# chengzhag/PanFusion

Measured on NVIDIA H100. Metric: denoise-steps/sec (512x1024 pano + 8x512^2 views, 50-step DDIM), higher is better.
Workload: dtype bf16

## Files before the change

### panfusion_b200/csrc/gemm_common.cuh

```cuda
#pragma once
#include "pf_common.cuh"

namespace pf {

constexpr int GEMM_BLOCK_M = 128;
constexpr int GEMM_BLOCK_K = 64;
constexpr int GEMM_WIN_SPAN = 8;
constexpr int GEMM_WIN_BYTES = (GEMM_BLOCK_M + GEMM_WIN_SPAN) * GEMM_BLOCK_K * 2;

struct GemmKernelParams {
  int M, N, kb_per_tap;
  int num_groups, num_units;
  int grp_first[PF_MAX_TAPS + 1];
  int grp_off[PF_MAX_TAPS];
  int tap_src[PF_MAX_TAPS];
  int a_rows, a_slots, slab_ring;
  unsigned long long grp_shifts[PF_MAX_TAPS];
  void* out;
  int out_ld;
  int out_f32;
  const float* bias;
  const float* rowbias;
  int rowbias_ld;
  int rows_per_group;
  const void* residual;
  int res_ld;
  int res_f32;
  int act;
  int map_mode, Hm, Wm, i0, j0, Hout, Wout;
  int osy, osx, oa, ob;
  int k_splits;
  float* ws;
  float* row_stats;
  int stat_slots;
  const float* ln_stats;
  int ln_slots;
  const float* ln_colsum;
  float ln_inv_k, ln_eps;
};

__device__ __forceinline__ void ln_row_coeffs(const GemmKernelParams& p, long long m, float& a, float& b) {
  const float4* st = reinterpret_cast<const float4*>(p.ln_stats) + m * (p.ln_slots >> 1);
  const int pairs = p.ln_slots >> 1;
  float s = 0.f, q = 0.f;
  for (int i0 = 0; i0 < pairs; i0 += 4) {
    float4 v[4];
#pragma unroll
    for (int u = 0; u < 4; ++u) v[u] = i0 + u < pairs ? __ldg(st + i0 + u) : make_float4(0.f, 0.f, 0.f, 0.f);
#pragma unroll
    for (int u = 0; u < 4; ++u) {
      s += v[u].x;
      q += v[u].y;
      s += v[u].z;
      q += v[u].w;
    }
  }
  const float mean = s * p.ln_inv_k;
  const float var = fmaxf(q * p.ln_inv_k - mean * mean, 0.f);
  a = rsqrtf(var + p.ln_eps);
  b = -mean * a;
}

__host__ __device__ constexpr int gemm_stage_bytes(int block_n) {
  return GEMM_BLOCK_M * GEMM_BLOCK_K * 2 + block_n * GEMM_BLOCK_K * 2;
}

}
```

### panfusion_b200/csrc/gemm_wgmma.cu

```cuda
#include <stdlib.h>

#include "gemm_common.cuh"
#include "wgmma.cuh"

namespace pf {

constexpr int GEMM_THREADS = 256;

constexpr int GEMM_SUB_BYTES = GEMM_BLOCK_M * 64;
constexpr int GEMM_SMEM_CORESIDENT = 228 * 1024 / 2 - 1024;

__host__ __device__ constexpr int gemm_acc_ld(int block_n) { return block_n + 4; }
__host__ __device__ constexpr int gemm_acc_bytes(int block_n) {
  return (GEMM_BLOCK_M * gemm_acc_ld(block_n) * 4 + 1023) / 1024 * 1024;
}
__host__ __device__ constexpr int gemm_ring_bytes(int block_n, int stages, bool epi_tma) {
  const int ring = stages * gemm_stage_bytes(block_n);
  const int epi = gemm_acc_bytes(block_n) + (epi_tma ? 2 * GEMM_SUB_BYTES : 0);
  return ((ring > epi ? ring : epi) + 1023) / 1024 * 1024;
}
__host__ __device__ constexpr int gemm_bar_bytes(int stages) { return (2 * stages * 12 + 15) / 16 * 16; }
__host__ __device__ constexpr int gemm_smem_bytes(int block_n, int stages, bool epi_tma) {
  return gemm_ring_bytes(block_n, stages, epi_tma) + gemm_bar_bytes(stages) +
         2 * block_n * 4 ;
}

template <int BLOCK_N, int STAGES, int CTAS, bool BF16, bool EPI_TMA>
__global__ void __launch_bounds__(GEMM_THREADS, CTAS)
gemm_taps_kernel(const __grid_constant__ CUtensorMap tmA, const __grid_constant__ CUtensorMap tmB,
                 const __grid_constant__ CUtensorMap tmC, const GemmKernelParams p) {
  constexpr int B_BYTES = BLOCK_N * GEMM_BLOCK_K * 2;
  constexpr int RING_BYTES = gemm_ring_bytes(BLOCK_N, STAGES, EPI_TMA);
  constexpr int ACC_LD = gemm_acc_ld(BLOCK_N);
  constexpr int NCH = BLOCK_N / 16;
  constexpr int NACC = BLOCK_N / 2;
  static_assert(BLOCK_N % 32 == 0 && BLOCK_N <= 256, "tile width");

  extern __shared__ __align__(1024) uint8_t smem[];
  if ((smem_u32(smem) & 1023u) != 0) __trap();
  float* sacc = reinterpret_cast<float*>(smem);
  uint8_t* staging = smem + gemm_acc_bytes(BLOCK_N);
  const int a_bytes = p.a_rows * (GEMM_BLOCK_K * 2);
  uint8_t* const b_ring = smem + p.a_slots * a_bytes;
  uint64_t* a_full = reinterpret_cast<uint64_t*>(smem + RING_BYTES);
  uint64_t* b_full = a_full + STAGES;
  uint32_t* a_rel = reinterpret_cast<uint32_t*>(b_full + STAGES);
  uint32_t* b_rel = a_rel + STAGES;
  float* s_bias = reinterpret_cast<float*>(smem + RING_BYTES + gemm_bar_bytes(STAGES));
  float* s_cs = s_bias + BLOCK_N;

  const int et = threadIdx.x;
  const int lane = et & 31;
  const int wg = et >> 7;
  const int n_tiles = p.N / BLOCK_N;
  const int n_tile = int(blockIdx.x) % n_tiles;
  const int m0 = (int(blockIdx.x) / n_tiles) * GEMM_BLOCK_M;
  const int n0 = n_tile * BLOCK_N;
  const int kpt = p.kb_per_tap;
  const int split = p.k_splits > 1 ? int(blockIdx.y) : 0;
  const int u_begin = (p.k_splits > 1) ? (int)((long long)split * p.num_units / p.k_splits) : 0;
  const int u_end = (p.k_splits > 1) ? (int)((long long)(split + 1) * p.num_units / p.k_splits) : p.num_units;
  auto first_slab = [&](int u) {
    const int gu = u / kpt, ku = u - gu * kpt;
    return p.grp_first[gu] * kpt + (ku ? ku * (p.grp_first[gu + 1] - p.grp_first[gu]) : 0);
  };
  const int s_begin = first_slab(u_begin), s_end = first_slab(u_end);

  if (et == 0) {
    tma_prefetch_desc(&tmA);
    tma_prefetch_desc(&tmB);
    for (int s = 0; s < STAGES; ++s) {
      mbar_init(&a_full[s], 1);
      mbar_init(&b_full[s], 1);
      a_rel[s] = b_rel[s] = 0u;
    }
    if constexpr (EPI_TMA) tma_prefetch_desc(&tmC);
    fence_barrier_init();
  }
  __syncthreads();

  auto locate = [&](int s, int& gs, int& ks, int& is) {
    gs = 0;
    while (s >= p.grp_first[gs + 1] * kpt) ++gs;
    const int taps = p.grp_first[gs + 1] - p.grp_first[gs];
    const int r = s - p.grp_first[gs] * kpt;
    ks = r / taps;
    is = p.grp_first[gs] + r - ks * taps;
  };
  auto load_a = [&](int slot, int ga, int ka, uint64_t* bar) {
    tma_load_2d(smem + slot * a_bytes, &tmA, bar, ka * GEMM_BLOCK_K, m0 + p.grp_off[ga]);
  };
  auto fill_a = [&](int slot, int ga, int ka) {
    mbar_expect_tx(&a_full[slot], a_bytes);
    load_a(slot, ga, ka, &a_full[slot]);
  };
  auto fill_b = [&](int slot, int gb, int kb, int ib) {
    mbar_expect_tx(&b_full[slot], B_BYTES + (p.slab_ring ? a_bytes : 0));
    if (p.slab_ring) load_a(slot, gb, kb, &b_full[slot]);
    tma_load_2d(b_ring + slot * B_BYTES, &tmB, &b_full[slot], (p.tap_src[ib] * kpt + kb) * GEMM_BLOCK_K, n0);
  };
  if (et == 0) {
    if (!p.slab_ring)
      for (int k = 0; k < p.a_slots && u_begin + k < u_end; ++k) {
        const int gu = (u_begin + k) / kpt;
        fill_a(k, gu, u_begin + k - gu * kpt);
      }
    for (int k = 0; k < STAGES && s_begin + k < s_end; ++k) {
      int gs, ks, is;
      locate(s_begin + k, gs, ks, is);
      fill_b(k, gs, ks, is);
    }
  }
  auto released_last = [](uint32_t* counter) {
    __threadfence_block();
    const uint32_t before = atomicAdd(counter, 1u);
    __threadfence_block();
    return (before & 1u) != 0u;
  };

  if (p.bias && et < BLOCK_N) s_bias[et] = __ldg(p.bias + n0 + et);
  if (p.ln_stats && et < BLOCK_N) s_cs[et] = __ldg(p.ln_colsum + n0 + et);
  {
    float acc[NACC];
#pragma unroll
    for (int i = 0; i < NACC; ++i) acc[i] = 0.f;
    int g = u_begin / kpt, kk = u_begin - g * kpt, t = 0;
    int gsize = p.grp_first[g + 1] - p.grp_first[g];
    uint64_t gshift = p.grp_shifts[g];
    int a_slot = 0, a_par = 0, b_slot = 0, b_par = 0;
    int gb = 0, kb = 0, ib = 0;
    if (s_begin + STAGES < s_end) locate(s_begin + STAGES, gb, kb, ib);
    int ib0 = p.grp_first[gb], ib_end = p.grp_first[gb + 1];
    int ua = u_begin + p.a_slots, ga = ua / kpt, ka = ua - ga * kpt;
    auto issue_slab = [&]() {
      if (!p.slab_ring && t == 0) mbar_wait(&a_full[a_slot], a_par);
      mbar_wait(&b_full[b_slot], b_par);
      const int shift = int(gshift >> (4 * t)) & 15;
      const uint32_t sa = smem_u32(smem + a_slot * a_bytes) + (shift + wg * 64) * (GEMM_BLOCK_K * 2);
      const uint64_t adesc = make_wgmma_desc(sa, 16, 1024, 1);
      const uint64_t bdesc = make_wgmma_desc(smem_u32(b_ring + b_slot * B_BYTES), 16, 1024, 1);
      wgmma_fence();
      fence_regs(acc);
#pragma unroll
      for (int k = 0; k < GEMM_BLOCK_K / 16; ++k)
        Wgmma<BLOCK_N, BF16>::ss(acc, adesc + 2 * k, bdesc + 2 * k, 1);
      wgmma_commit();
      fence_regs(acc);
    };
    issue_slab();
    for (int s = s_begin + 1; s < s_end; ++s) {
      if (++b_slot == STAGES) {
        b_slot = 0;
        b_par ^= 1;
      }
      const bool new_window = ++t == gsize;
      if (new_window) {
        t = 0;
        if (++kk == kpt) {
          kk = 0;
          ++g;
          gsize = p.grp_first[g + 1] - p.grp_first[g];
          gshift = p.grp_shifts[g];
        }
        if (++a_slot == p.a_slots) {
          a_slot = 0;
          a_par ^= 1;
        }
      }
      issue_slab();
      wgmma_wait<1>();
      fence_regs(acc);
      const bool load_b = s - 1 + STAGES < s_end;
      const bool load_a = !p.slab_ring && new_window && ua < u_end;
      if ((et & 127) == 0) {
        const int bs = (b_slot ? b_slot : STAGES) - 1;
        if (load_b && released_last(&b_rel[bs])) fill_b(bs, gb, kb, ib);
        const int as = (a_slot ? a_slot : p.a_slots) - 1;
        if (load_a && released_last(&a_rel[as])) fill_a(as, ga, ka);
      }
      if (load_b && ++ib == ib_end) {
        if (++kb == kpt) {
          kb = 0;
          ++gb;
          ib0 = ib_end;
          ib_end = gb < p.num_groups ? p.grp_first[gb + 1] : ib_end;
        }
        ib = ib0;
      }
      if (load_a) {
        ++ua;
        if (++ka == kpt) {
          ka = 0;
          ++ga;
        }
      }
    }
    wgmma_wait<0>();
    fence_regs(acc);
    named_bar_sync(1, GEMM_THREADS);
    const int r0 = wg * 64 + ((et >> 5) & 3) * 16 + (lane >> 2);
    const int cb = 2 * (lane & 3);
#pragma unroll
    for (int j = 0; j < BLOCK_N / 8; ++j) {
      *reinterpret_cast<float2*>(sacc + r0 * ACC_LD + 8 * j + cb) = make_float2(acc[4 * j], acc[4 * j + 1]);
      *reinterpret_cast<float2*>(sacc + (r0 + 8) * ACC_LD + 8 * j + cb) = make_float2(acc[4 * j + 2], acc[4 * j + 3]);
    }
  }
  named_bar_sync(1, GEMM_THREADS);

  const int row = et & 127;
  const int half = et >> 7;
  const float* arow = sacc + row * ACC_LD;
  const int m = m0 + row;
  bool valid = m < p.M;
  long long orow = m;
  int group = 0;
  if (p.map_mode == 1) {
    const int hw = p.Hm * p.Wm;
    const int img = m / hw;
    const int r = m - img * hw;
    const int i = r / p.Wm;
    const int j = r - i * p.Wm;
    valid = valid && i >= p.i0 && i < p.i0 + p.Hout && j >= p.j0 && j < p.j0 + p.Wout;
    orow = ((long long)img * p.Hout * p.osy + (i - p.i0) * p.osy + p.oa) * (p.Wout * p.osx) + (j - p.j0) * p.osx + p.ob;
    group = img;
  } else if (p.rowbias) {
    group = m / p.rows_per_group;
  }
  if (!valid) group = 0;
  float ln_a = 1.f, ln_b = 0.f;
  if (p.ln_stats && m < p.M) ln_row_coeffs(p, m, ln_a, ln_b);
  const float* rb_base = p.rowbias ? p.rowbias + (long long)group * p.rowbias_ld + n0 : nullptr;
  auto load16 = [&](int c, float (&o)[16]) {
#pragma unroll
    for (int e = 0; e < 4; ++e) {
      const float4 t = *reinterpret_cast<const float4*>(arow + c + 4 * e);
      o[4 * e] = t.x;
      o[4 * e + 1] = t.y;
      o[4 * e + 2] = t.z;
      o[4 * e + 3] = t.w;
    }
  };

  if (p.k_splits > 1) {
    if (m < p.M) {
      float* wrow = p.ws + ((long long)split * p.M + m) * p.N + n0;
#pragma unroll 1
      for (int ci = half; ci < NCH; ci += 2) {
        float o[16];
        load16(ci * 16, o);
        float4* dst = reinterpret_cast<float4*>(wrow + ci * 16);
#pragma unroll
        for (int e = 0; e < 4; ++e) dst[e] = make_float4(o[4 * e], o[4 * e + 1], o[4 * e + 2], o[4 * e + 3]);
      }
    }
  } else if constexpr (EPI_TMA) {
    static_assert(NCH % 2 == 0, "a sub-tile is one chunk of each of a row's two threads");
    const uint32_t sw = uint32_t((row >> 1) & 3);
    float st_s = 0.f, st_q = 0.f;
    const uint16_t* res_row =
        p.residual && m < p.M ? static_cast<const uint16_t*>(p.residual) + (long long)m * p.res_ld + n0 : nullptr;
#pragma unroll 1
    for (int ci = half; ci < NCH; ci += 2) {
      const int c = ci * 16;
      uint4 r0 = make_uint4(0u, 0u, 0u, 0u), r1 = r0;
      if (res_row) {
        r0 = __ldg(reinterpret_cast<const uint4*>(res_row + c));
        r1 = __ldg(reinterpret_cast<const uint4*>(res_row + c) + 1);
      }
      float o[16];
      load16(c, o);
      if (p.ln_stats) {
#pragma unroll
        for (int e = 0; e < 16; ++e) o[e] = fmaf(o[e], ln_a, s_cs[c + e] * ln_b);
      }
      if (p.bias) {
#pragma unroll
        for (int e = 0; e < 16; ++e) o[e] += s_bias[c + e];
      }
      if (rb_base) {
#pragma unroll
        for (int e = 0; e < 16; ++e) o[e] += __ldg(rb_base + c + e);
      }
      if (p.act == PF_ACT_SILU) {
#pragma unroll
        for (int e = 0; e < 16; ++e) o[e] = silu_f(o[e]);
      } else if (p.act == PF_ACT_GELU) {
#pragma unroll
        for (int e = 0; e < 16; ++e) o[e] = gelu_erf_f(o[e]);
      } else if (p.act == PF_ACT_QUICK_GELU) {
#pragma unroll
        for (int e = 0; e < 16; ++e) o[e] = quick_gelu_f(o[e]);
      }
      const int sub = c >> 5;
      uint8_t* sbuf = staging + (sub & 1) * GEMM_SUB_BYTES;
      uint8_t* srow = sbuf + row * 64;
      const uint32_t q0 = uint32_t((c >> 4) & 1) * 2;
      uint4* s0 = reinterpret_cast<uint4*>(srow + (((q0 + 0) ^ sw) << 4));
      uint4* s1 = reinterpret_cast<uint4*>(srow + (((q0 + 1) ^ sw) << 4));
      if (p.residual) {
        float2 f;
        f = unpack2<BF16>(r0.x); o[0] += f.x; o[1] += f.y;
        f = unpack2<BF16>(r0.y); o[2] += f.x; o[3] += f.y;
        f = unpack2<BF16>(r0.z); o[4] += f.x; o[5] += f.y;
        f = unpack2<BF16>(r0.w); o[6] += f.x; o[7] += f.y;
        f = unpack2<BF16>(r1.x); o[8] += f.x; o[9] += f.y;
        f = unpack2<BF16>(r1.y); o[10] += f.x; o[11] += f.y;
        f = unpack2<BF16>(r1.z); o[12] += f.x; o[13] += f.y;
        f = unpack2<BF16>(r1.w); o[14] += f.x; o[15] += f.y;
      }
      if (p.row_stats) {
#pragma unroll
        for (int e = 0; e < 16; ++e) {
          st_s += o[e];
          st_q = fmaf(o[e], o[e], st_q);
        }
      }
      *s0 = make_uint4(pack2<BF16>(o[0], o[1]), pack2<BF16>(o[2], o[3]), pack2<BF16>(o[4], o[5]),
                       pack2<BF16>(o[6], o[7]));
      *s1 = make_uint4(pack2<BF16>(o[8], o[9]), pack2<BF16>(o[10], o[11]), pack2<BF16>(o[12], o[13]),
                       pack2<BF16>(o[14], o[15]));
      fence_proxy_async_smem();
      if (et == 0) tma_store_wait_read();
      named_bar_sync(1, GEMM_THREADS);
      if (et == 0) {
        tma_store_2d(&tmC, sbuf, n0 + sub * 32, m0);
        tma_store_commit();
      }
    }
    if (p.row_stats && m < p.M)
      reinterpret_cast<float2*>(p.row_stats)[(long long)m * p.stat_slots + n_tile * 2 + half] = make_float2(st_s, st_q);
    if (et == 0) tma_store_wait_read();
  } else if (p.act == PF_ACT_GEGLU) {
    constexpr int HALF_N = BLOCK_N / 2;
    const int on0 = n_tile * HALF_N;
    if constexpr (HALF_N % 16 == 0) {
#pragma unroll 1
      for (int c = half * 16; c < HALF_N; c += 32) {
        if (!valid) break;
        float va[16], vg[16], o[16], ba[16], bg[16];
        load16(c, va);
        load16(HALF_N + c, vg);
        if (p.bias) {
#pragma unroll
          for (int e = 0; e < 4; ++e) {
            *reinterpret_cast<float4*>(ba + 4 * e) = *reinterpret_cast<const float4*>(s_bias + c + 4 * e);
            *reinterpret_cast<float4*>(bg + 4 * e) = *reinterpret_cast<const float4*>(s_bias + HALF_N + c + 4 * e);
          }
        } else {
#pragma unroll
          for (int e = 0; e < 16; ++e) ba[e] = bg[e] = 0.f;
        }
        if (p.ln_stats) {
#pragma unroll
          for (int e = 0; e < 16; ++e) {
            va[e] = fmaf(va[e], ln_a, s_cs[c + e] * ln_b);
            vg[e] = fmaf(vg[e], ln_a, s_cs[HALF_N + c + e] * ln_b);
          }
        }
#pragma unroll
        for (int e = 0; e < 16; e += 2)
          geglu_pair(va[e], va[e + 1], vg[e], vg[e + 1], ba[e], ba[e + 1], bg[e], bg[e + 1], o[e], o[e + 1]);
        if (p.out_f32) {
          float4* dst = reinterpret_cast<float4*>(static_cast<float*>(p.out) + orow * p.out_ld + on0 + c);
#pragma unroll
          for (int e = 0; e < 4; ++e) dst[e] = make_float4(o[4 * e], o[4 * e + 1], o[4 * e + 2], o[4 * e + 3]);
        } else {
          uint4* dst = reinterpret_cast<uint4*>(static_cast<uint16_t*>(p.out) + orow * p.out_ld + on0 + c);
          dst[0] = make_uint4(pack2<BF16>(o[0], o[1]), pack2<BF16>(o[2], o[3]), pack2<BF16>(o[4], o[5]),
                              pack2<BF16>(o[6], o[7]));
          dst[1] = make_uint4(pack2<BF16>(o[8], o[9]), pack2<BF16>(o[10], o[11]), pack2<BF16>(o[12], o[13]),
                              pack2<BF16>(o[14], o[15]));
        }
      }
    }
  } else if (valid) {
#pragma unroll 1
    for (int ci = half; ci < NCH; ci += 2) {
      const int c = ci * 16;
      float o[16];
      load16(c, o);
      if (p.bias) {
#pragma unroll
        for (int e = 0; e < 16; ++e) o[e] += s_bias[c + e];
      }
      if (rb_base) {
#pragma unroll
        for (int e = 0; e < 4; ++e) {
          const float4 t = __ldg(reinterpret_cast<const float4*>(rb_base + c) + e);
          o[4 * e] += t.x;
          o[4 * e + 1] += t.y;
          o[4 * e + 2] += t.z;
          o[4 * e + 3] += t.w;
        }
      }
      if (p.act == PF_ACT_SILU) {
#pragma unroll
        for (int e = 0; e < 16; ++e) o[e] = silu_f(o[e]);
      } else if (p.act == PF_ACT_GELU) {
#pragma unroll
        for (int e = 0; e < 16; ++e) o[e] = gelu_erf_f(o[e]);
      } else if (p.act == PF_ACT_QUICK_GELU) {
#pragma unroll
        for (int e = 0; e < 16; ++e) o[e] = quick_gelu_f(o[e]);
      }
      if (p.residual) {
        if (p.res_f32) {
          const float4* r4 =
              reinterpret_cast<const float4*>(static_cast<const float*>(p.residual) + orow * p.res_ld + n0 + c);
#pragma unroll
          for (int e = 0; e < 4; ++e) {
            const float4 t = r4[e];
            o[4 * e] += t.x;
            o[4 * e + 1] += t.y;
            o[4 * e + 2] += t.z;
            o[4 * e + 3] += t.w;
          }
        } else {
          const uint4* r16 =
              reinterpret_cast<const uint4*>(static_cast<const uint16_t*>(p.residual) + orow * p.res_ld + n0 + c);
          const uint4 r0 = __ldg(r16), r1 = __ldg(r16 + 1);
          float2 f;
          f = unpack2<BF16>(r0.x); o[0] += f.x; o[1] += f.y;
          f = unpack2<BF16>(r0.y); o[2] += f.x; o[3] += f.y;
          f = unpack2<BF16>(r0.z); o[4] += f.x; o[5] += f.y;
          f = unpack2<BF16>(r0.w); o[6] += f.x; o[7] += f.y;
          f = unpack2<BF16>(r1.x); o[8] += f.x; o[9] += f.y;
          f = unpack2<BF16>(r1.y); o[10] += f.x; o[11] += f.y;
          f = unpack2<BF16>(r1.z); o[12] += f.x; o[13] += f.y;
          f = unpack2<BF16>(r1.w); o[14] += f.x; o[15] += f.y;
        }
      }
      if (p.out_f32) {
        float4* dst = reinterpret_cast<float4*>(static_cast<float*>(p.out) + orow * p.out_ld + n0 + c);
#pragma unroll
        for (int e = 0; e < 4; ++e) dst[e] = make_float4(o[4 * e], o[4 * e + 1], o[4 * e + 2], o[4 * e + 3]);
      } else {
        uint4* dst = reinterpret_cast<uint4*>(static_cast<uint16_t*>(p.out) + orow * p.out_ld + n0 + c);
        dst[0] = make_uint4(pack2<BF16>(o[0], o[1]), pack2<BF16>(o[2], o[3]), pack2<BF16>(o[4], o[5]),
                            pack2<BF16>(o[6], o[7]));
        dst[1] = make_uint4(pack2<BF16>(o[8], o[9]), pack2<BF16>(o[10], o[11]), pack2<BF16>(o[12], o[13]),
                            pack2<BF16>(o[14], o[15]));
      }
    }
  }
}

template <bool BF16>
__global__ void __launch_bounds__(256) splitk_reduce_kernel(const GemmKernelParams p) {
  const int vecs = p.N / 8;
  const long long idx = (long long)blockIdx.x * blockDim.x + threadIdx.x;
  if (idx >= (long long)p.M * vecs) return;
  const int m = int(idx / vecs), c = int(idx % vecs) * 8;
  bool valid = true;
  long long orow = m;
  int group = 0;
  if (p.map_mode == 1) {
    const int hw = p.Hm * p.Wm;
    const int img = m / hw;
    const int r = m - img * hw;
    const int i = r / p.Wm;
    const int j = r - i * p.Wm;
    valid = i >= p.i0 && i < p.i0 + p.Hout && j >= p.j0 && j < p.j0 + p.Wout;
    orow = ((long long)img * p.Hout * p.osy + (i - p.i0) * p.osy + p.oa) * (p.Wout * p.osx) + (j - p.j0) * p.osx + p.ob;
    group = img;
  } else if (p.rowbias) {
    group = m / p.rows_per_group;
  }
  if (!valid) return;
  float o[8];
#pragma unroll
  for (int e = 0; e < 8; ++e) o[e] = 0.f;
  for (int sp = 0; sp < p.k_splits; ++sp) {
    const float4* w4 = reinterpret_cast<const float4*>(p.ws + ((long long)sp * p.M + m) * p.N + c);
    const float4 a = __ldcs(w4), b = __ldcs(w4 + 1);
    o[0] += a.x; o[1] += a.y; o[2] += a.z; o[3] += a.w;
    o[4] += b.x; o[5] += b.y; o[6] += b.z; o[7] += b.w;
  }
  if (p.bias) {
#pragma unroll
    for (int e = 0; e < 8; ++e) o[e] += __ldg(p.bias + c + e);
  }
  if (p.rowbias) {
    const float* rb = p.rowbias + (long long)group * p.rowbias_ld + c;
#pragma unroll
    for (int e = 0; e < 8; ++e) o[e] += __ldg(rb + e);
  }
  if (p.act == PF_ACT_SILU) {
#pragma unroll
    for (int e = 0; e < 8; ++e) o[e] = silu_f(o[e]);
  } else if (p.act == PF_ACT_GELU) {
#pragma unroll
    for (int e = 0; e < 8; ++e) o[e] = gelu_erf_f(o[e]);
  } else if (p.act == PF_ACT_QUICK_GELU) {
#pragma unroll
    for (int e = 0; e < 8; ++e) o[e] = quick_gelu_f(o[e]);
  }
  if (p.residual) {
    if (p.res_f32) {
      const float4* r4 = reinterpret_cast<const float4*>(static_cast<const float*>(p.residual) + orow * p.res_ld + c);
      const float4 a = r4[0], b = r4[1];
      o[0] += a.x; o[1] += a.y; o[2] += a.z; o[3] += a.w;
      o[4] += b.x; o[5] += b.y; o[6] += b.z; o[7] += b.w;
    } else {
      const uint4 t = *reinterpret_cast<const uint4*>(static_cast<const uint16_t*>(p.residual) + orow * p.res_ld + c);
      float2 f;
      f = unpack2<BF16>(t.x); o[0] += f.x; o[1] += f.y;
      f = unpack2<BF16>(t.y); o[2] += f.x; o[3] += f.y;
      f = unpack2<BF16>(t.z); o[4] += f.x; o[5] += f.y;
      f = unpack2<BF16>(t.w); o[6] += f.x; o[7] += f.y;
    }
  }
  if (p.out_f32) {
    float4* dst = reinterpret_cast<float4*>(static_cast<float*>(p.out) + orow * p.out_ld + c);
    dst[0] = make_float4(o[0], o[1], o[2], o[3]);
    dst[1] = make_float4(o[4], o[5], o[6], o[7]);
  } else {
    *reinterpret_cast<uint4*>(static_cast<uint16_t*>(p.out) + orow * p.out_ld + c) =
        make_uint4(pack2<BF16>(o[0], o[1]), pack2<BF16>(o[2], o[3]), pack2<BF16>(o[4], o[5]), pack2<BF16>(o[6], o[7]));
  }
}

template <int BLOCK_N, int STAGES, int CTAS, bool EPI_TMA>
static int launch_gemm(const pf_gemm_args* a, GemmKernelParams kp, cudaStream_t st) {
  const int a_slots = (gemm_ring_bytes(BLOCK_N, STAGES, EPI_TMA) - STAGES * BLOCK_N * GEMM_BLOCK_K * 2) /
                      (kp.a_rows * GEMM_BLOCK_K * 2);
  kp.a_slots = a_slots < STAGES ? a_slots : STAGES;
  static_assert(gemm_ring_bytes(BLOCK_N, STAGES, EPI_TMA) - STAGES * BLOCK_N * GEMM_BLOCK_K * 2 >= 2 * GEMM_WIN_BYTES,
                "two A windows next to the B boxes");
  CUtensorMap tmA, tmB, tmC;
  {
    uint64_t dims[2] = {(uint64_t)a->Kc, (uint64_t)a->a_rows};
    uint64_t str[1] = {(uint64_t)a->a_ld * 2};
    uint32_t box[2] = {GEMM_BLOCK_K, (uint32_t)kp.a_rows};
    int rc = make_tmap(&tmA, a->dtype, 2, a->A, dims, str, box, 128);
    if (rc) return rc;
  }
  {
    uint64_t dims[2] = {(uint64_t)a->Kc * a->num_taps, (uint64_t)a->N};
    uint64_t str[1] = {(uint64_t)a->b_ld * 2};
    uint32_t box[2] = {GEMM_BLOCK_K, (uint32_t)BLOCK_N};
    int rc = make_tmap(&tmB, a->dtype, 2, a->B, dims, str, box, 128);
    if (rc) return rc;
  }
  tmC = tmA;
  if constexpr (EPI_TMA) {
    uint64_t dims[2] = {(uint64_t)a->N, (uint64_t)a->M};
    uint32_t box[2] = {32, GEMM_BLOCK_M};
    uint64_t str[1] = {(uint64_t)a->out_ld * 2};
    int rc = make_tmap(&tmC, a->dtype, 2, a->out, dims, str, box, 64);
    if (rc) return rc;
  }
  constexpr int SMEM = gemm_smem_bytes(BLOCK_N, STAGES, EPI_TMA);
  static_assert(SMEM <= 227 * 1024, "shared memory budget of one H100 CTA");
  static_assert(CTAS == 1 || SMEM <= GEMM_SMEM_CORESIDENT, "two CTAs per SM: 113 KB of shared memory each");
  const int m_tiles = (a->M + GEMM_BLOCK_M - 1) / GEMM_BLOCK_M;
  const dim3 grid(m_tiles * (a->N / BLOCK_N), kp.k_splits > 1 ? kp.k_splits : 1);
  const int bf = a->dtype == PF_BF16;
  auto kern = bf ? gemm_taps_kernel<BLOCK_N, STAGES, CTAS, true, EPI_TMA>
                 : gemm_taps_kernel<BLOCK_N, STAGES, CTAS, false, EPI_TMA>;
  static bool attr_set[2] = {false, false};
  if (!attr_set[bf]) {
    int rc = check_cuda(cudaFuncSetAttribute(kern, cudaFuncAttributeMaxDynamicSharedMemorySize, SMEM),
                        "cudaFuncSetAttribute(gemm)");
    if (rc) return rc;
    int resident = 0;
    rc = check_cuda(cudaOccupancyMaxActiveBlocksPerMultiprocessor(&resident, kern, GEMM_THREADS, SMEM),
                    "cudaOccupancyMaxActiveBlocksPerMultiprocessor(gemm)");
    if (rc) return rc;
    if (resident < CTAS) {
      set_error("gemm_taps_kernel<%d, %d, %s>: %d CTA(s) per SM fit, built for %d", BLOCK_N, STAGES,
                EPI_TMA ? "tma" : "direct", resident, CTAS);
      return PF_ERR_UNSUPPORTED;
    }
    attr_set[bf] = true;
  }
  kern<<<grid, GEMM_THREADS, SMEM, st>>>(tmA, tmB, tmC, kp);
  PF_CHECK_LAUNCH("gemm_taps_kernel");
  return PF_OK;
}

static int resolve_block_n(const pf_gemm_args* a) {
  int bn = (a->block_n & 0xffff) ? (a->block_n & 0xffff) : pf_gemm_pick_block_n(a->N, a->act);
  if (a->row_stats_out) bn = pf_gemm_pick_block_n(a->N, a->act);
  if ((a->row_stats_out || a->ln_stats) && a->act != PF_ACT_GEGLU && bn == 256) bn = 128;
  return bn;
}

}

extern "C" int pf_gemm_row_stats_slots(const pf_gemm_args* a) {
  if (!a || a->N <= 0) return 0;
  pf_gemm_args producer = *a;
  static float dummy;
  producer.row_stats_out = &dummy;
  const int bn = pf::resolve_block_n(&producer);
  return bn > 0 && a->N % bn == 0 ? 2 * (a->N / bn) : 0;
}

extern "C" int pf_gemm_pick_block_n(int N, int act) {
  if (act == PF_ACT_GEGLU && N % 256 == 0) return 256;
  if (N % 160 == 0) return 160;
  if (N % 128 == 0) return 128;
  if (N % 64 == 0) return 64;
  return 0;
}

extern "C" int pf_gemm_splitk_plan(const pf_gemm_args* a) {
  if (!a || a->act == PF_ACT_GEGLU || a->M <= 0 || a->N <= 0 || a->Kc <= 0) return 1;
  const int bn = pf_gemm_pick_block_n(a->N, a->act);
  if (!bn) return 1;
  const long long tiles = (long long)((a->M + 127) / 128) * (a->N / bn);
  const int num_kb = a->Kc / 64 * a->num_taps;
  const int sms = pf::sm_count();
  if (tiles > sms / 2 || num_kb < 64) return 1;
  int s = (int)((sms + tiles - 1) / tiles);
  const int max_by_k = num_kb / 16;
  if (s > max_by_k) s = max_by_k;
  if (s > 16) s = 16;
  return s < 2 ? 1 : s;
}

extern "C" int pf_gemm_taps(const pf_gemm_args* a, void* stream) {
  using namespace pf;
  PF_CHECK_ARG(a != nullptr, "pf_gemm_taps: null args");
  PF_CHECK_ARG(a->dtype == PF_BF16 || a->dtype == PF_F16, "pf_gemm_taps: dtype must be PF_F16 or PF_BF16");
  PF_CHECK_ARG(a->A && a->B && a->out, "pf_gemm_taps: null operand");
  PF_CHECK_ARG(a->M > 0 && a->N > 0 && a->Kc > 0, "pf_gemm_taps: empty problem M=%d N=%d Kc=%d", a->M, a->N, a->Kc);
  PF_CHECK_ARG(a->Kc % GEMM_BLOCK_K == 0, "pf_gemm_taps: Kc=%d must be a multiple of 64", a->Kc);
  PF_CHECK_ARG(a->num_taps >= 1 && a->num_taps <= PF_MAX_TAPS, "pf_gemm_taps: num_taps=%d out of range", a->num_taps);
  PF_CHECK_ARG(a->a_ld % 8 == 0 && a->b_ld % 8 == 0 && a->a_ld >= a->Kc && a->b_ld >= a->Kc * a->num_taps,
               "pf_gemm_taps: bad leading dims a_ld=%d b_ld=%d", a->a_ld, a->b_ld);
  PF_CHECK_ARG((reinterpret_cast<uintptr_t>(a->A) & 15) == 0 && (reinterpret_cast<uintptr_t>(a->B) & 15) == 0 &&
                   (reinterpret_cast<uintptr_t>(a->out) & 15) == 0,
               "pf_gemm_taps: operands must be 16-byte aligned");
  PF_CHECK_ARG((reinterpret_cast<uintptr_t>(a->residual) & 15) == 0, "pf_gemm_taps: residual must be 16-byte aligned");
  PF_CHECK_ARG(!a->rowbias || ((reinterpret_cast<uintptr_t>(a->rowbias) & 15) == 0 && a->rowbias_ld % 4 == 0),
               "pf_gemm_taps: rowbias must be 16-byte aligned with rowbias_ld %% 4 == 0 (rowbias_ld=%d)", a->rowbias_ld);
  PF_CHECK_ARG((reinterpret_cast<uintptr_t>(a->splitk_ws) & 15) == 0, "pf_gemm_taps: splitk_ws must be 16-byte aligned");
  PF_CHECK_ARG((reinterpret_cast<uintptr_t>(a->row_stats_out) & 7) == 0,
               "pf_gemm_taps: row_stats_out must be 8-byte aligned");
  PF_CHECK_ARG(a->out_dtype == PF_F32 || a->out_dtype == a->dtype, "pf_gemm_taps: out_dtype must be f32 or dtype");
  PF_CHECK_ARG(!a->residual || a->res_dtype == PF_F32 || a->res_dtype == a->dtype,
               "pf_gemm_taps: res_dtype must be f32 or dtype");
  PF_CHECK_ARG(a->act >= PF_ACT_NONE && a->act <= PF_ACT_QUICK_GELU, "pf_gemm_taps: unknown act %d", a->act);
  int bn = pf::resolve_block_n(a);
  PF_CHECK_ARG(bn == 64 || bn == 128 || bn == 160 || bn == 256, "pf_gemm_taps: unsupported block_n %d (N=%d)", bn, a->N);
  PF_CHECK_ARG(a->N % bn == 0, "pf_gemm_taps: N=%d not a multiple of block_n=%d", a->N, bn);
  const int n_out = a->act == PF_ACT_GEGLU ? a->N / 2 : a->N;
  PF_CHECK_ARG(a->out_ld % 8 == 0 && a->out_ld >= n_out, "pf_gemm_taps: bad out_ld %d", a->out_ld);
  PF_CHECK_ARG(!a->residual || (a->res_ld % 8 == 0 && a->res_ld >= n_out), "pf_gemm_taps: bad res_ld %d", a->res_ld);
  PF_CHECK_ARG(!(a->act == PF_ACT_GEGLU && (a->residual || a->rowbias)),
               "pf_gemm_taps: GEGLU epilogue takes no residual/rowbias");
  if (a->map_mode == 1) {
    PF_CHECK_ARG(a->Hm > 0 && a->Wm > 0 && a->Hout > 0 && a->Wout > 0 && a->M % (a->Hm * a->Wm) == 0,
                 "pf_gemm_taps: bad image map Hm=%d Wm=%d M=%d", a->Hm, a->Wm, a->M);
    PF_CHECK_ARG(a->out_sy >= 0 && a->out_sx >= 0 && a->out_a >= 0 && a->out_b >= 0 &&
                     a->out_a < (a->out_sy > 0 ? a->out_sy : 1) && a->out_b < (a->out_sx > 0 ? a->out_sx : 1),
                 "pf_gemm_taps: bad output scatter (%d,%d) phase (%d,%d)", a->out_sy, a->out_sx, a->out_a, a->out_b);
    PF_CHECK_ARG((a->out_sy <= 1 && a->out_sx <= 1) || !a->residual, "pf_gemm_taps: the scattered output map takes no residual");
  } else {
    PF_CHECK_ARG(a->map_mode == 0, "pf_gemm_taps: unknown map_mode %d", a->map_mode);
    PF_CHECK_ARG(!a->rowbias || a->rows_per_group > 0, "pf_gemm_taps: rowbias needs rows_per_group");
  }

  GemmKernelParams kp;
  kp.M = a->M;
  kp.N = a->N;
  kp.kb_per_tap = a->Kc / GEMM_BLOCK_K;
  int order[PF_MAX_TAPS];
  for (int t = 0; t < a->num_taps; ++t) {
    int k = t;
    for (; k > 0 && a->tap_off[order[k - 1]] > a->tap_off[t]; --k) order[k] = order[k - 1];
    order[k] = t;
  }
  kp.num_groups = 0;
  for (int k = 0; k < PF_MAX_TAPS; ++k) kp.grp_shifts[k] = 0;
  int span = 0;
  for (int k = 0; k < a->num_taps; ++k) {
    const int off = a->tap_off[order[k]];
    if (k == 0 || (long long)off - kp.grp_off[kp.num_groups - 1] > GEMM_WIN_SPAN) {
      kp.grp_first[kp.num_groups] = k;
      kp.grp_off[kp.num_groups++] = off;
    }
    const int shift = off - kp.grp_off[kp.num_groups - 1];
    kp.grp_shifts[kp.num_groups - 1] |= uint64_t(shift) << (4 * (k - kp.grp_first[kp.num_groups - 1]));
    kp.tap_src[k] = order[k];
    span = span > shift ? span : shift;
  }
  kp.grp_first[kp.num_groups] = a->num_taps;
  kp.num_units = kp.num_groups * kp.kb_per_tap;
  kp.a_rows = GEMM_BLOCK_M + (span ? GEMM_WIN_SPAN : 0);
  kp.slab_ring = kp.num_groups == a->num_taps;
  kp.out = a->out;
  kp.out_ld = a->out_ld;
  kp.out_f32 = a->out_dtype == PF_F32;
  kp.bias = a->bias;
  kp.rowbias = a->rowbias;
  kp.rowbias_ld = a->rowbias_ld;
  kp.rows_per_group = a->rows_per_group > 0 ? a->rows_per_group : 1;
  kp.residual = a->residual;
  kp.res_ld = a->res_ld;
  kp.res_f32 = a->res_dtype == PF_F32;
  kp.act = a->act;
  kp.map_mode = a->map_mode;
  kp.Hm = a->Hm;
  kp.Wm = a->Wm;
  kp.i0 = a->i0;
  kp.j0 = a->j0;
  kp.Hout = a->Hout;
  kp.Wout = a->Wout;
  kp.osy = a->out_sy > 0 ? a->out_sy : 1;
  kp.osx = a->out_sx > 0 ? a->out_sx : 1;
  kp.oa = a->out_a;
  kp.ob = a->out_b;
  kp.k_splits = a->k_splits > 1 ? a->k_splits : 1;
  kp.ws = a->splitk_ws;
  kp.row_stats = a->row_stats_out;
  kp.stat_slots = 2 * (a->N / bn);
  kp.ln_stats = a->ln_stats;
  kp.ln_slots = a->ln_slots;
  kp.ln_colsum = a->ln_colsum;
  kp.ln_inv_k = 1.0f / float((long long)a->Kc * a->num_taps);
  kp.ln_eps = a->ln_eps;
  PF_CHECK_ARG(kp.k_splits == 1 || (a->splitk_ws && a->act != PF_ACT_GEGLU && kp.k_splits <= kp.num_units),
               "pf_gemm_taps: split-K needs a workspace, no GEGLU and k_splits <= (tap window, channel slab) units");
  const bool fused_ln = a->row_stats_out || a->ln_stats;
  if (fused_ln) {
    PF_CHECK_ARG(kp.k_splits == 1, "pf_gemm_taps: fused LayerNorm does not combine with split-K");
    PF_CHECK_ARG(!a->ln_stats || (a->ln_colsum && a->ln_slots > 0 && a->ln_slots % 2 == 0 && a->ln_eps > 0.f &&
                                  (reinterpret_cast<uintptr_t>(a->ln_stats) & 15) == 0),
                 "pf_gemm_taps: ln_stats needs ln_colsum, ln_slots and ln_eps");
    const bool plain16 = a->map_mode == 0 && a->out_dtype == a->dtype && (!a->residual || a->res_dtype == a->dtype);
    PF_CHECK_ARG(a->act == PF_ACT_GEGLU ? !a->row_stats_out : plain16,
                 "pf_gemm_taps: fused LayerNorm needs the plain row map with 16-bit output (consumer: or GEGLU)");
  }
  cudaStream_t st = static_cast<cudaStream_t>(stream);
  if (kp.k_splits > 1) {
    int rc;
    switch (bn) {
      case 64: rc = launch_gemm<64, 8, 1, false>(a, kp, st); break;
      case 128: rc = launch_gemm<128, 6, 1, false>(a, kp, st); break;
      case 160: rc = launch_gemm<160, 5, 1, false>(a, kp, st); break;
      default: rc = launch_gemm<256, 4, 1, false>(a, kp, st); break;
    }
    if (rc) return rc;
    const long long total = (long long)a->M * (a->N / 8);
    if (a->dtype == PF_BF16) splitk_reduce_kernel<true><<<(unsigned)((total + 255) / 256), 256, 0, st>>>(kp);
    else splitk_reduce_kernel<false><<<(unsigned)((total + 255) / 256), 256, 0, st>>>(kp);
    PF_CHECK_LAUNCH("splitk_reduce_kernel");
    return PF_OK;
  }
  const bool epi_tma = a->map_mode == 0 && a->out_dtype == a->dtype && a->act != PF_ACT_GEGLU &&
                       (!a->residual || a->res_dtype == a->dtype) && bn != 256;
  if (epi_tma) {
    switch (bn) {
      case 64: return launch_gemm<64, 4, 2, true>(a, kp, st);
      case 128: return launch_gemm<128, 3, 2, true>(a, kp, st);
      case 160: return launch_gemm<160, 3, 2, true>(a, kp, st);
    }
  }
  switch (bn) {
    case 64: return launch_gemm<64, 4, 2, false>(a, kp, st);
    case 128: return launch_gemm<128, 3, 2, false>(a, kp, st);
    case 160: return launch_gemm<160, 3, 2, false>(a, kp, st);
    case 256: return launch_gemm<256, 4, 1, false>(a, kp, st);
  }
  return PF_ERR_UNSUPPORTED;
}
```

Before: 22.01.

## Add warp-specialized persistent GEMM kernel for single-tap linear layers

Adds a dedicated persistent GEMM kernel for plain single-tap linear layers (no rowbias, 16-bit output). It has one TMA producer warp, two consumer warpgroups, and a helper warp group that computes fused LayerNorm row coefficients, with register rebalancing via setmaxnreg. The residual tile is prefetched by TMA during the mainloop, and GEGLU is applied in registers for BLOCK_N=256. The aim is to overlap loads, LN-stat reduction and the epilogue with the MMA and to cut epilogue shared-memory traffic. In exchange it adds a second code path whose stage counts and tiling differ from the generic kernel.

```diff
diff --git a/panfusion_b200/csrc/gemm_common.cuh b/panfusion_b200/csrc/gemm_common.cuh
--- a/panfusion_b200/csrc/gemm_common.cuh
+++ b/panfusion_b200/csrc/gemm_common.cuh
@@ -65,4 +65,6 @@
   return GEMM_BLOCK_M * GEMM_BLOCK_K * 2 + block_n * GEMM_BLOCK_K * 2;
 }
 
+int launch_gemm_linear(const pf_gemm_args* a, const GemmKernelParams& kp, int bn, cudaStream_t st);
+
 }
diff --git a/panfusion_b200/csrc/gemm_linear.cu b/panfusion_b200/csrc/gemm_linear.cu
--- /dev/null
+++ b/panfusion_b200/csrc/gemm_linear.cu
@@ -0,0 +1,360 @@
+#include "gemm_common.cuh"
+#include "wgmma.cuh"
+
+namespace pf {
+
+constexpr int LIN_THREADS = 384;
+constexpr int LIN_SUB_COLS = 32;
+constexpr int LIN_SUB_BYTES = 64 * LIN_SUB_COLS * 2;
+constexpr int LIN_RES_SUB_BYTES = GEMM_BLOCK_M * LIN_SUB_COLS * 2;
+
+__host__ __device__ constexpr int lin_out_cols(int block_n, bool geglu) { return geglu ? block_n / 2 : block_n; }
+__host__ __device__ constexpr int lin_ring_bytes(int block_n, int stages) { return stages * gemm_stage_bytes(block_n); }
+__host__ __device__ constexpr int lin_staging_bytes(int block_n, bool geglu) {
+  return 2 * 64 * lin_out_cols(block_n, geglu) * 2;
+}
+__host__ __device__ constexpr int lin_res_bytes(int block_n, bool geglu) { return geglu ? 0 : GEMM_BLOCK_M * block_n * 2; }
+__host__ __device__ constexpr int lin_smem_bytes(int block_n, int stages, bool geglu) {
+  return lin_ring_bytes(block_n, stages) + lin_staging_bytes(block_n, geglu) + lin_res_bytes(block_n, geglu) +
+         2 * GEMM_BLOCK_M * 8  + (2 * stages + 6) * 8;
+}
+
+__device__ __forceinline__ void setmaxnreg_inc232() { asm volatile("setmaxnreg.inc.sync.aligned.u32 232;\n" ::: "memory"); }
+__device__ __forceinline__ void setmaxnreg_dec40() { asm volatile("setmaxnreg.dec.sync.aligned.u32 40;\n" ::: "memory"); }
+
+__device__ __forceinline__ uint32_t lin_sw_off(int r, int c, int rows) {
+  return uint32_t((c >> 5) * rows * 64 + r * 64 + ((((c & 31) >> 3) ^ ((r >> 1) & 3)) << 4) + (c & 7) * 2);
+}
+
+template <int BLOCK_N, int STAGES, bool GEGLU, bool BF16>
+__global__ void __launch_bounds__(LIN_THREADS, 1)
+gemm_linear_kernel(const __grid_constant__ CUtensorMap tmA, const __grid_constant__ CUtensorMap tmB,
+                   const __grid_constant__ CUtensorMap tmC, const __grid_constant__ CUtensorMap tmR,
+                   const GemmKernelParams p) {
+  constexpr int A_BYTES = GEMM_BLOCK_M * GEMM_BLOCK_K * 2;
+  constexpr int B_BYTES = BLOCK_N * GEMM_BLOCK_K * 2;
+  constexpr int STAGE_BYTES = A_BYTES + B_BYTES;
+  constexpr int NACC = BLOCK_N / 2;
+  constexpr int OUT_N = lin_out_cols(BLOCK_N, GEGLU);
+  constexpr int NSUB = OUT_N / LIN_SUB_COLS;
+  static_assert(OUT_N % LIN_SUB_COLS == 0, "output tile in 32-column sub-tiles");
+  static_assert(!GEGLU || BLOCK_N == 256, "GEGLU in registers: value and gate columns 128 apart");
+
+  extern __shared__ __align__(1024) uint8_t smem[];
+  if ((smem_u32(smem) & 1023u) != 0) __trap();
+  uint8_t* const staging = smem + lin_ring_bytes(BLOCK_N, STAGES);
+  uint8_t* const res_tile = staging + lin_staging_bytes(BLOCK_N, GEGLU);
+  float2* const ln_coef = reinterpret_cast<float2*>(res_tile + lin_res_bytes(BLOCK_N, GEGLU));
+  uint64_t* const full = reinterpret_cast<uint64_t*>(ln_coef + 2 * GEMM_BLOCK_M);
+  uint64_t* const empty = full + STAGES;
+  uint64_t* const res_full = empty + STAGES;
+  uint64_t* const res_empty = res_full + 1;
+  uint64_t* const ln_full = res_empty + 1;
+  uint64_t* const ln_empty = ln_full + 2;
+
+  const int n_tiles = p.N / BLOCK_N;
+  const int tiles = (p.M + GEMM_BLOCK_M - 1) / GEMM_BLOCK_M * n_tiles;
+  const int kslabs = p.kb_per_tap;
+  const bool has_res = p.residual != nullptr;
+  const int wg = threadIdx.x >> 7;
+
+  if (threadIdx.x == 0) {
+    for (int s = 0; s < STAGES; ++s) {
+      mbar_init(&full[s], 1);
+      mbar_init(&empty[s], 2);
+    }
+    mbar_init(res_full, 1);
+    mbar_init(res_empty, 2);
+    for (int s = 0; s < 2; ++s) {
+      mbar_init(&ln_full[s], 96);
+      mbar_init(&ln_empty[s], 2);
+    }
+    fence_barrier_init();
+  }
+  __syncthreads();
+
+  if (wg == 2) {
+    setmaxnreg_dec40();
+    if (threadIdx.x >= 288) {
+      if (!p.ln_stats) return;
+      int i = 0;
+      for (int tile = blockIdx.x; tile < tiles; tile += gridDim.x, ++i) {
+        const int m0 = (tile / n_tiles) * GEMM_BLOCK_M;
+        mbar_wait(&ln_empty[i & 1], ((i >> 1) & 1) ^ 1);
+        for (int r = threadIdx.x - 288; r < GEMM_BLOCK_M; r += 96) {
+          float a = 1.f, b = 0.f;
+          if (m0 + r < p.M) ln_row_coeffs(p, m0 + r, a, b);
+          ln_coef[(i & 1) * GEMM_BLOCK_M + r] = make_float2(a, b);
+        }
+        mbar_arrive(&ln_full[i & 1]);
+      }
+      return;
+    }
+    if (threadIdx.x != 256) return;
+    tma_prefetch_desc(&tmA);
+    tma_prefetch_desc(&tmB);
+    if (has_res) tma_prefetch_desc(&tmR);
+    int slot = 0, par = 0, res_par = 0;
+    const int res_after = (kslabs < STAGES ? kslabs : STAGES) - 1;
+    for (int tile = blockIdx.x; tile < tiles; tile += gridDim.x) {
+      const int n0 = (tile % n_tiles) * BLOCK_N;
+      const int m0 = (tile / n_tiles) * GEMM_BLOCK_M;
+      for (int k = 0; k < kslabs; ++k) {
+        mbar_wait(&empty[slot], par ^ 1);
+        mbar_expect_tx(&full[slot], STAGE_BYTES);
+        uint8_t* st = smem + slot * STAGE_BYTES;
+        tma_load_2d(st, &tmA, &full[slot], k * GEMM_BLOCK_K, m0 + p.grp_off[0]);
+        tma_load_2d(st + A_BYTES, &tmB, &full[slot], k * GEMM_BLOCK_K, n0);
+        if (++slot == STAGES) {
+          slot = 0;
+          par ^= 1;
+        }
+        if (!GEGLU && has_res && k == res_after) {
+          mbar_wait(res_empty, res_par ^ 1);
+          mbar_expect_tx(res_full, lin_res_bytes(BLOCK_N, GEGLU));
+#pragma unroll 1
+          for (int s = 0; s < BLOCK_N / LIN_SUB_COLS; ++s)
+            tma_load_2d(res_tile + s * LIN_RES_SUB_BYTES, &tmR, res_full, n0 + s * LIN_SUB_COLS, m0);
+          res_par ^= 1;
+        }
+      }
+    }
+    return;
+  }
+
+  setmaxnreg_inc232();
+  const int et = threadIdx.x & 127;
+  const int lane = threadIdx.x & 31;
+  const int rl = ((et >> 5) << 4) + (lane >> 2);
+  const int cb = 2 * (lane & 3);
+  uint8_t* const my_staging = staging + wg * (NSUB * LIN_SUB_BYTES);
+  if (et == 0) tma_prefetch_desc(&tmC);
+  int slot = 0, par = 0, res_par = 0;
+  float acc[NACC];
+
+  for (int tile = blockIdx.x, ti = 0; tile < tiles; tile += gridDim.x, ++ti) {
+    const int n_tile = tile % n_tiles;
+    const int n0 = n_tile * BLOCK_N;
+    const int m0 = (tile / n_tiles) * GEMM_BLOCK_M;
+
+#pragma unroll
+    for (int i = 0; i < NACC; ++i) acc[i] = 0.f;
+    auto issue_slab = [&]() {
+      mbar_wait(&full[slot], par);
+      const uint32_t sa = smem_u32(smem + slot * STAGE_BYTES) + wg * 64 * (GEMM_BLOCK_K * 2);
+      const uint64_t adesc = make_wgmma_desc(sa, 16, 1024, 1);
+      const uint64_t bdesc = make_wgmma_desc(smem_u32(smem + slot * STAGE_BYTES + A_BYTES), 16, 1024, 1);
+      wgmma_fence();
+      fence_regs(acc);
+#pragma unroll
+      for (int k = 0; k < GEMM_BLOCK_K / 16; ++k)
+        Wgmma<BLOCK_N, BF16>::ss(acc, adesc + 2 * k, bdesc + 2 * k, 1);
+      wgmma_commit();
+      fence_regs(acc);
+    };
+    issue_slab();
+    int prev = slot;
+    if (++slot == STAGES) {
+      slot = 0;
+      par ^= 1;
+    }
+    for (int k = 1; k < kslabs; ++k) {
+      issue_slab();
+      wgmma_wait<1>();
+      fence_regs(acc);
+      if (et == 0) mbar_arrive(&empty[prev]);
+      prev = slot;
+      if (++slot == STAGES) {
+        slot = 0;
+        par ^= 1;
+      }
+    }
+    wgmma_wait<0>();
+    fence_regs(acc);
+    if (et == 0) mbar_arrive(&empty[prev]);
+
+    const int ma = m0 + wg * 64 + rl, mb = ma + 8;
+    if (p.ln_stats) {
+      mbar_wait(&ln_full[ti & 1], (ti >> 1) & 1);
+      const float2 ca = ln_coef[(ti & 1) * GEMM_BLOCK_M + wg * 64 + rl];
+      const float2 cc = ln_coef[(ti & 1) * GEMM_BLOCK_M + wg * 64 + rl + 8];
+      const float la = ca.x, lb = ca.y, ha = cc.x, hb = cc.y;
+#pragma unroll
+      for (int j = 0; j < BLOCK_N / 8; ++j) {
+        const float cs0 = __ldg(p.ln_colsum + n0 + 8 * j + cb), cs1 = __ldg(p.ln_colsum + n0 + 8 * j + cb + 1);
+        acc[4 * j] = fmaf(acc[4 * j], la, cs0 * lb);
+        acc[4 * j + 1] = fmaf(acc[4 * j + 1], la, cs1 * lb);
+        acc[4 * j + 2] = fmaf(acc[4 * j + 2], ha, cs0 * hb);
+        acc[4 * j + 3] = fmaf(acc[4 * j + 3], ha, cs1 * hb);
+      }
+    }
+    if constexpr (GEGLU) {
+#pragma unroll
+      for (int j = 0; j < OUT_N / 8; ++j) {
+        float ba0 = 0.f, ba1 = 0.f, bg0 = 0.f, bg1 = 0.f;
+        if (p.bias) {
+          ba0 = __ldg(p.bias + n0 + 8 * j + cb);
+          ba1 = __ldg(p.bias + n0 + 8 * j + cb + 1);
+          bg0 = __ldg(p.bias + n0 + OUT_N + 8 * j + cb);
+          bg1 = __ldg(p.bias + n0 + OUT_N + 8 * j + cb + 1);
+        }
+        constexpr int G = 4 * (OUT_N / 8);
+        geglu_pair(acc[4 * j], acc[4 * j + 1], acc[G + 4 * j], acc[G + 4 * j + 1], ba0, ba1, bg0, bg1, acc[4 * j],
+                   acc[4 * j + 1]);
+        geglu_pair(acc[4 * j + 2], acc[4 * j + 3], acc[G + 4 * j + 2], acc[G + 4 * j + 3], ba0, ba1, bg0, bg1,
+                   acc[4 * j + 2], acc[4 * j + 3]);
+      }
+    } else {
+      if (p.bias) {
+#pragma unroll
+        for (int j = 0; j < BLOCK_N / 8; ++j) {
+          const float b0 = __ldg(p.bias + n0 + 8 * j + cb), b1 = __ldg(p.bias + n0 + 8 * j + cb + 1);
+          acc[4 * j] += b0;
+          acc[4 * j + 1] += b1;
+          acc[4 * j + 2] += b0;
+          acc[4 * j + 3] += b1;
+        }
+      }
+      if (p.act == PF_ACT_SILU) {
+#pragma unroll
+        for (int i = 0; i < NACC; ++i) acc[i] = silu_f(acc[i]);
+      } else if (p.act == PF_ACT_GELU) {
+#pragma unroll
+        for (int i = 0; i < NACC; ++i) acc[i] = gelu_erf_f(acc[i]);
+      } else if (p.act == PF_ACT_QUICK_GELU) {
+#pragma unroll
+        for (int i = 0; i < NACC; ++i) acc[i] = quick_gelu_f(acc[i]);
+      }
+      if (has_res) {
+        mbar_wait(res_full, res_par);
+        res_par ^= 1;
+#pragma unroll
+        for (int j = 0; j < BLOCK_N / 8; ++j) {
+          const float2 ra = unpack2<BF16>(
+              *reinterpret_cast<const uint32_t*>(res_tile + lin_sw_off(wg * 64 + rl, 8 * j + cb, GEMM_BLOCK_M)));
+          const float2 rb = unpack2<BF16>(
+              *reinterpret_cast<const uint32_t*>(res_tile + lin_sw_off(wg * 64 + rl + 8, 8 * j + cb, GEMM_BLOCK_M)));
+          acc[4 * j] += ra.x;
+          acc[4 * j + 1] += ra.y;
+          acc[4 * j + 2] += rb.x;
+          acc[4 * j + 3] += rb.y;
+        }
+      }
+      if (p.row_stats) {
+        float s[2][2] = {{0.f, 0.f}, {0.f, 0.f}}, q[2][2] = {{0.f, 0.f}, {0.f, 0.f}};
+#pragma unroll
+        for (int j = 0; j < BLOCK_N / 8; ++j) {
+          const int h = (j >> 1) & 1;
+#pragma unroll
+          for (int e = 0; e < 2; ++e) {
+            s[0][h] += acc[4 * j + e];
+            q[0][h] = fmaf(acc[4 * j + e], acc[4 * j + e], q[0][h]);
+            s[1][h] += acc[4 * j + 2 + e];
+            q[1][h] = fmaf(acc[4 * j + 2 + e], acc[4 * j + 2 + e], q[1][h]);
+          }
+        }
+#pragma unroll
+        for (int r = 0; r < 2; ++r)
+#pragma unroll
+          for (int h = 0; h < 2; ++h) {
+            s[r][h] += __shfl_xor_sync(0xffffffffu, s[r][h], 1);
+            q[r][h] += __shfl_xor_sync(0xffffffffu, q[r][h], 1);
+            s[r][h] += __shfl_xor_sync(0xffffffffu, s[r][h], 2);
+            q[r][h] += __shfl_xor_sync(0xffffffffu, q[r][h], 2);
+          }
+        if ((lane & 3) < 2) {
+          const int h = lane & 1;
+          float2* st = reinterpret_cast<float2*>(p.row_stats) + n_tile * 2 + h;
+          if (ma < p.M) st[(long long)ma * p.stat_slots] = make_float2(h ? s[0][1] : s[0][0], h ? q[0][1] : q[0][0]);
+          if (mb < p.M) st[(long long)mb * p.stat_slots] = make_float2(h ? s[1][1] : s[1][0], h ? q[1][1] : q[1][0]);
+        }
+      }
+    }
+
+    if (et == 0) tma_store_wait_read();
+    named_bar_sync(1 + wg, 128);
+    if (et == 0) {
+      if (!GEGLU && has_res) mbar_arrive(res_empty);
+      if (p.ln_stats) mbar_arrive(&ln_empty[ti & 1]);
+    }
+#pragma unroll
+    for (int j = 0; j < OUT_N / 8; ++j) {
+      *reinterpret_cast<uint32_t*>(my_staging + lin_sw_off(rl, 8 * j + cb, 64)) = pack2<BF16>(acc[4 * j], acc[4 * j + 1]);
+      *reinterpret_cast<uint32_t*>(my_staging + lin_sw_off(rl + 8, 8 * j + cb, 64)) =
+          pack2<BF16>(acc[4 * j + 2], acc[4 * j + 3]);
+    }
+    fence_proxy_async_smem();
+    named_bar_sync(1 + wg, 128);
+    if (et == 0) {
+#pragma unroll 1
+      for (int s = 0; s < NSUB; ++s)
+        tma_store_2d(&tmC, my_staging + s * LIN_SUB_BYTES, n_tile * OUT_N + s * LIN_SUB_COLS, m0 + wg * 64);
+      tma_store_commit();
+    }
+  }
+  if (et == 0) tma_store_wait_read();
+}
+
+template <int BLOCK_N, int STAGES, bool GEGLU>
+static int launch_linear(const pf_gemm_args* a, const GemmKernelParams& kp, cudaStream_t st) {
+  constexpr int OUT_N = lin_out_cols(BLOCK_N, GEGLU);
+  CUtensorMap tmA, tmB, tmC, tmR;
+  {
+    uint64_t dims[2] = {(uint64_t)a->Kc, (uint64_t)a->a_rows};
+    uint64_t str[1] = {(uint64_t)a->a_ld * 2};
+    uint32_t box[2] = {GEMM_BLOCK_K, GEMM_BLOCK_M};
+    int rc = make_tmap(&tmA, a->dtype, 2, a->A, dims, str, box, 128);
+    if (rc) return rc;
+  }
+  {
+    uint64_t dims[2] = {(uint64_t)a->Kc, (uint64_t)a->N};
+    uint64_t str[1] = {(uint64_t)a->b_ld * 2};
+    uint32_t box[2] = {GEMM_BLOCK_K, (uint32_t)BLOCK_N};
+    int rc = make_tmap(&tmB, a->dtype, 2, a->B, dims, str, box, 128);
+    if (rc) return rc;
+  }
+  {
+    uint64_t dims[2] = {(uint64_t)(a->N / BLOCK_N * OUT_N), (uint64_t)a->M};
+    uint64_t str[1] = {(uint64_t)a->out_ld * 2};
+    uint32_t box[2] = {LIN_SUB_COLS, 64};
+    int rc = make_tmap(&tmC, a->dtype, 2, a->out, dims, str, box, 64);
+    if (rc) return rc;
+  }
+  tmR = tmC;
+  if (a->residual) {
+    uint64_t dims[2] = {(uint64_t)a->N, (uint64_t)a->M};
+    uint64_t str[1] = {(uint64_t)a->res_ld * 2};
+    uint32_t box[2] = {LIN_SUB_COLS, GEMM_BLOCK_M};
+    int rc = make_tmap(&tmR, a->dtype, 2, a->residual, dims, str, box, 64);
+    if (rc) return rc;
+  }
+  constexpr int SMEM = lin_smem_bytes(BLOCK_N, STAGES, GEGLU);
+  static_assert(SMEM <= 227 * 1024, "shared memory budget of one H100 CTA");
+  const int bf = a->dtype == PF_BF16;
+  auto kern = bf ? gemm_linear_kernel<BLOCK_N, STAGES, GEGLU, true> : gemm_linear_kernel<BLOCK_N, STAGES, GEGLU, false>;
+  static bool attr_set[2] = {false, false};
+  if (!attr_set[bf]) {
+    int rc = check_cuda(cudaFuncSetAttribute(kern, cudaFuncAttributeMaxDynamicSharedMemorySize, SMEM),
+                        "cudaFuncSetAttribute(gemm_linear)");
+    if (rc) return rc;
+    attr_set[bf] = true;
+  }
+  const long long tiles = (long long)((a->M + GEMM_BLOCK_M - 1) / GEMM_BLOCK_M) * (a->N / BLOCK_N);
+  const int sms = sm_count();
+  const unsigned grid = (unsigned)(tiles < sms ? tiles : sms);
+  kern<<<grid, LIN_THREADS, SMEM, st>>>(tmA, tmB, tmC, tmR, kp);
+  PF_CHECK_LAUNCH("gemm_linear_kernel");
+  return PF_OK;
+}
+
+int launch_gemm_linear(const pf_gemm_args* a, const GemmKernelParams& kp, int bn, cudaStream_t st) {
+  if (a->act == PF_ACT_GEGLU) return bn == 256 ? launch_linear<256, 4, true>(a, kp, st) : PF_ERR_UNSUPPORTED;
+  switch (bn) {
+    case 64: return launch_linear<64, 8, false>(a, kp, st);
+    case 128: return launch_linear<128, 5, false>(a, kp, st);
+    case 160: return launch_linear<160, 4, false>(a, kp, st);
+  }
+  return PF_ERR_UNSUPPORTED;
+}
+
+}
diff --git a/panfusion_b200/csrc/gemm_wgmma.cu b/panfusion_b200/csrc/gemm_wgmma.cu
--- a/panfusion_b200/csrc/gemm_wgmma.cu
+++ b/panfusion_b200/csrc/gemm_wgmma.cu
@@ -751,6 +751,9 @@
     PF_CHECK_LAUNCH("splitk_reduce_kernel");
     return PF_OK;
   }
+  const bool plain16 = a->map_mode == 0 && a->out_dtype == a->dtype && (!a->residual || a->res_dtype == a->dtype);
+  if (a->num_taps == 1 && plain16 && !a->rowbias && (a->act == PF_ACT_GEGLU) == (bn == 256))
+    return launch_gemm_linear(a, kp, bn, st);
   const bool epi_tma = a->map_mode == 0 && a->out_dtype == a->dtype && a->act != PF_ACT_GEGLU &&
                        (!a->residual || a->res_dtype == a->dtype) && bn != 256;
   if (epi_tma) {
```

Result: faster. 23.14 (median of 6 runs) (+5.1%).
